# bblinn2017/inverse_path_tracer

Hardware: AMD Instinct MI355X
Metric: Msamples/sec fwd + grad-Msamples/sec, 512² Cornell 64spp, 1/2/4/8 GPU (higher is better)
Workload: dtype f32; 1 GPU; C2: CornellBox-Empty-CO.obj, 512x512, 64 spp, max_bounces=4; one frame per step tiled over the ranks as interleaved rows (fwd); adjoint dL/dKd of the rank's rows + RCCL all-reduce of the gradient (grad, --full); 3 frames in flight (consecutive steps round-robin over 3 HIP streams; one stream: secondary.serial); streams=3, width=512, height=512, spp=64, max_bounces=4, triangles=18, parallelism=interleaved row tiles x1

## Files before the change

inverse_path_tracer_amd/csrc/ipt_device.h:

```cpp
#pragma once
#include <hip/hip_runtime.h>
#include <stdint.h>

#include "scene_layout.h"

namespace ipt {
namespace dev {

typedef __attribute__((address_space(3))) float lds_f32;
typedef __attribute__((address_space(3))) double lds_f64;
typedef __attribute__((address_space(1))) float gbl_f32;
typedef __attribute__((address_space(1))) double gbl_f64;
typedef float v4f __attribute__((ext_vector_type(4)));
typedef __attribute__((address_space(3))) v4f lds_v4;
typedef __attribute__((address_space(1))) v4f gbl_v4;

constexpr float kMinDotUp = 0x1.a36e30p-14f;
constexpr float kEpsUp = 0x1.47ae16p-7f;
constexpr float kPRR = 0.9f;
constexpr float kPiF = 3.14159265358979323846f;
constexpr float kInvPiF = (float)(1.0 / 3.14159265358979323846);
constexpr double kPi = 3.14159265358979323846;

#ifndef IPT_DIV_CONST
// ... 1024 lines not shown
  if (M && lane == (int)__builtin_ctzll(__ballot(1))) atomicAdd(&g_bvh_stats[5], 1ull);
#endif
  while (M) {
#ifdef IPT_BVH_STATS
    if (lane == (int)__builtin_ctzll(__ballot(1))) atomicAdd(&g_bvh_stats[6], 1ull);
#endif
    uint64_t Mr = M;
    int src = -1;
#pragma unroll
    for (int k = 0; k < 8; ++k) {
      if (Mr) {
        const int idx = __builtin_ctzll(Mr);
        Mr &= Mr - 1;
        src = (g == k) ? idx : src;
      }
    }
    const uint64_t taken = M & ~Mr;
    M = Mr;
    const int sa = (src < 0 ? lane : src) << 2;
    const V3 gp = mk(bperm_f(sa, p.x), bperm_f(sa, p.y), bperm_f(sa, p.z));
    const V3 gd = mk(bperm_f(sa, d.x), bperm_f(sa, d.y), bperm_f(sa, d.z));
    float gt = bperm_f(sa, bt);
    int gi = __builtin_amdgcn_ds_bpermute(sa, bi);
    if (src >= 0) {
      coop_traverse<SHADOW>(C, gp, gd, gt, gi);
    }
    const int ra = (8 * lane_rank64(taken)) << 2;
    const float rt = bperm_f(ra, gt);
    const int ri = __builtin_amdgcn_ds_bpermute(ra, gi);
    if ((taken >> lane) & 1ull) {
      bt = rt;
      bi = ri;
    }
  }
}

__device__ __forceinline__ V3 shading_normal(const TriGeom &g, V3 q) {
  if (g.flags & GEOM_AXIS_FLAT) return mk(g.vn[0][0], g.vn[0][1], g.vn[0][2]);
  const V3 v0 = mk(g.v[0][0], g.v[0][1], g.v[0][2]);
  const V3 v1 = mk(g.v[1][0], g.v[1][1], g.v[1][2]);
  const V3 v2 = mk(g.v[2][0], g.v[2][1], g.v[2][2]);
  const V3 c0 = cross3(sub(v1, q), sub(v2, q));
  const V3 c1 = cross3(sub(v2, q), sub(v0, q));
  const V3 c2 = cross3(sub(v0, q), sub(v1, q));
  const float w0 = (0.5f * sqrtf(dot3(c0, c0))) / g.area;
  const float w1 = (0.5f * sqrtf(dot3(c1, c1))) / g.area;
  const float w2 = (0.5f * sqrtf(dot3(c2, c2))) / g.area;
  const V3 n = mk(fmaf(g.vn[2][0], w2, fmaf(g.vn[1][0], w1, g.vn[0][0] * w0)),
                  fmaf(g.vn[2][1], w2, fmaf(g.vn[1][1], w1, g.vn[0][1] * w0)),
                  fmaf(g.vn[2][2], w2, fmaf(g.vn[1][2], w1, g.vn[0][2] * w0)));
  return unit(n);
}

__device__ __forceinline__ void camera_ray(const float *cam, const float *org, Rng &st, int r, int c, int W, int H,
                                           float rcW, float rcH, V3 &p, V3 &d) {
  const float u0 = uniform(st), u1 = uniform(st);
  const float nx = 2.f * ((float)c + u0), ny = 2.f * ((float)r + u1);
  const float x = (rcW != 0.f ? nx * rcW : div_inrange(nx, (float)W)) - 1.f;
  const float y = 1.f - (rcH != 0.f ? ny * rcH : div_inrange(ny, (float)H));
  const V3 d0 = unit_in_range(mk(x, y, 1.f));
  float dr[3];
#pragma unroll
  for (int i = 0; i < 3; ++i) {
    const float *M = cam + 4 * i;
    dr[i] = fmaf(M[3], 0.f, fmaf(M[2], d0.z, fmaf(M[1], d0.y, M[0] * d0.x)));
  }
  p = mk(org[0], org[1], org[2]);
  d = unit(mk(dr[0], dr[1], dr[2]));
}

__device__ inline float phong(float shin, V3 nrm, V3 w, V3 wi) {
  const float dn = dot3(nrm, wi);
  const V3 refl = mk(fmaf(2.f * dn, nrm.x, -wi.x), fmaf(2.f * dn, nrm.y, -wi.y), fmaf(2.f * dn, nrm.z, -wi.z));
  const float pw = pow_f(dot3(refl, w), shin);
  const float mx = pw > 0.f ? pw : 0.f;
  return (float)((((double)(shin + 2.f)) / 2.0 / kPi) * (double)mx);
}

}
}
```

inverse_path_tracer_amd/csrc/ipt_hip.hip:

```cpp
#include <hip/hip_runtime.h>

#include <algorithm>
#include <atomic>
#include <cmath>
#include <cstdio>
#include <cstdlib>
#include <cstring>
#include <mutex>
#include <string>
#include <vector>

#include "bvh.h"
#include "gpu_api.h"
#include "ipt_device.h"

namespace ipt {

static thread_local std::string g_gpu_err;
void gpu_set_error(const std::string &e) { g_gpu_err = e; }
const char *gpu_last_error() { return g_gpu_err.c_str(); }
static std::atomic<int> g_fail_launches{0};
void gpu_debug_fail_launches(int n) { g_fail_launches.store(n > 0 ? n : 0); }
static std::atomic<int> g_adju_pool{0}, g_adju_lds{0};
void gpu_debug_adju_ring(int pool_chunks, int lds_slots) {
// ... 204 lines not shown
  return BVH || IPT_BF_BIG > 1;
}
template <bool GUIDED>
__device__ __forceinline__ void chunk_range(const TraceArgs &a, uint64_t g, uint64_t units, uint64_t &start,
                                            uint64_t &end) {
  const uint64_t nb = a.chunk_big_n;
  uint64_t len;
  if (!GUIDED || g < nb) {
    start = g * a.chunk;
    len = a.chunk;
  } else {
    start = nb * a.chunk + (g - nb) * a.chunk_small;
    len = a.chunk_small;
  }
  end = start + len < units ? start + len : units;
}

__device__ __forceinline__ void grab_failed(uint32_t *word, uint32_t c, uint32_t grabs) {
  if (c + 1u == grabs) __hip_atomic_store(word, 0u, __ATOMIC_RELAXED, __HIP_MEMORY_SCOPE_AGENT);
}

__device__ __forceinline__ uint64_t item_pixel(const TraceArgs &a, uint64_t w) {
  uint64_t lp, sj;
  item_split(a, w, lp, sj);
  int r, c;
  local_rc(a, lp, r, c);
  if (a.idx32) return (uint32_t)r * (uint32_t)a.W + (uint32_t)c;
  return (uint64_t)r * (uint64_t)a.W + (uint64_t)c;
}

using namespace dev;
typedef __attribute__((address_space(3))) uint32_t lds_u32;

__device__ __forceinline__ void item_ray_ls(const TraceArgs &a, uint64_t seed, uint64_t lp, uint64_t sj, Rng &st, V3 &p,
                                            V3 &d, int &r, int &c) {
  local_rc(a, lp, r, c);
  uint64_t g;
  if (a.idx32) {
    const uint32_t pixel = (uint32_t)r * (uint32_t)a.W + (uint32_t)c;
    g = (uint64_t)pixel * (uint32_t)a.spp + sj;
  } else {
    g = ((uint64_t)r * (uint64_t)a.W + (uint64_t)c) * (uint64_t)a.spp + sj;
  }
  rng_init(st, seed + g);
  camera_ray(a.cam, a.cam_org, st, r, c, a.W, a.H, a.rc_W, a.rc_H, p, d);
}
__device__ __forceinline__ void item_ray(const TraceArgs &a, uint64_t seed, uint64_t w, Rng &st, V3 &p, V3 &d, int &r,
                                         int &c) {
  uint64_t lp, sj;
  item_split(a, w, lp, sj);
  item_ray_ls(a, seed, lp, sj, st, p, d, r, c);
}

#ifndef IPT_MIN_BLOCKS_FWD
#define IPT_MIN_BLOCKS_FWD 5
#endif
#ifndef IPT_MIN_BLOCKS_ADJ
#define IPT_MIN_BLOCKS_ADJ 5
#endif
#ifndef IPT_MIN_BLOCKS_ADJU
#define IPT_MIN_BLOCKS_ADJU 5
#endif
#ifndef IPT_MIN_BLOCKS_ADJW
#define IPT_MIN_BLOCKS_ADJW 6
#endif
#ifndef IPT_ADJW_LANE_LDS
#define IPT_ADJW_LANE_LDS 1
#endif
#ifndef IPT_MIN_BLOCKS_GRAPH
#define IPT_MIN_BLOCKS_GRAPH 0
#endif
#ifndef IPT_MIN_BLOCKS_BVH
#define IPT_MIN_BLOCKS_BVH 4
#endif
#ifndef IPT_MIN_BLOCKS_BVH_ADJ
#define IPT_MIN_BLOCKS_BVH_ADJ 2
#endif
#ifndef IPT_MIN_BLOCKS_BVH_ADJU
#define IPT_MIN_BLOCKS_BVH_ADJU 4
#endif
#ifndef IPT_MIN_BLOCKS_BVH_FWD
#define IPT_MIN_BLOCKS_BVH_FWD 5
#endif
template <int MODE, bool BVH>
constexpr int min_blocks() {
  return BVH ? (MODE == MODE_ADJU ? IPT_MIN_BLOCKS_BVH_ADJU
                                  : (is_adj<MODE>() ? IPT_MIN_BLOCKS_BVH_ADJ
                                                    : (is_fwd<MODE>() ? IPT_MIN_BLOCKS_BVH_FWD : IPT_MIN_BLOCKS_BVH)))
             : (is_fwd<MODE>() ? IPT_MIN_BLOCKS_FWD
                                : (MODE == MODE_ADJU   ? IPT_MIN_BLOCKS_ADJU
                                   : MODE == MODE_ADJW ? IPT_MIN_BLOCKS_ADJW
                                                       : (is_adj<MODE>() ? IPT_MIN_BLOCKS_ADJ : IPT_MIN_BLOCKS_GRAPH)));
}
#ifndef IPT_GRAPH_LDS_KB
#define IPT_GRAPH_LDS_KB 64
#endif
#ifndef IPT_ADJ_PIXEL_MAJOR
#define IPT_ADJ_PIXEL_MAJOR 1
#endif
#ifndef IPT_GRAPH_PIXEL_MAJOR
#define IPT_GRAPH_PIXEL_MAJOR 1
#endif
#define IPT_TRACE_BOUNDS __attribute__((amdgpu_flat_work_group_size(1, kBlock), amdgpu_waves_per_eu(min_blocks<MODE, BVH>() ? min_blocks<MODE, BVH>() : 1)))
#ifdef IPT_PHASE_TIMING
constexpr int kPhaseWords = 26;
__device__ unsigned long long g_phase_cycles[kPhaseWords];
// ... 322 lines not shown
  if (hipMemcpyFromSymbol(out, HIP_SYMBOL(g_phase_cycles), kPhaseWords * sizeof(unsigned long long)) != hipSuccess)
    return -1;
  unsigned long long z[kPhaseWords] = {};
  return hipMemcpyToSymbol(HIP_SYMBOL(g_phase_cycles), z, sizeof z) == hipSuccess ? 0 : -1;
}
#endif

#ifdef IPT_BVH_STATS
extern "C" int ipt_debug_bvh_stats(unsigned long long *out) {
  if (hipMemcpyFromSymbol(out, HIP_SYMBOL(g_bvh_stats), kBvhStats * sizeof(unsigned long long)) != hipSuccess)
    return -1;
  unsigned long long z[kBvhStats] = {0};
  return hipMemcpyToSymbol(HIP_SYMBOL(g_bvh_stats), z, sizeof z) == hipSuccess ? 0 : -1;
}
#endif

const HostScene &gpu_host(const GpuScene *s) { return s->host; }
HostScene &gpu_host_mut(GpuScene *s) { return s->host; }

template <typename T>
static int upload(T **dst, const std::vector<T> &v) {
  const size_t n = std::max<size_t>(v.size(), 1) * sizeof(T);
  HIP_TRY(hipMalloc(reinterpret_cast<void **>(dst), n));
  if (!v.empty()) HIP_TRY(hipMemcpy(*dst, v.data(), v.size() * sizeof(T), hipMemcpyHostToDevice));
  return 0;
}

template <typename T>
static int upload_as_f4(float4 **dst, const std::vector<T> &v) {
  static_assert(sizeof(T) % sizeof(float4) == 0, "record is not a whole number of float4");
  HIP_TRY(hipMalloc(reinterpret_cast<void **>(dst), std::max<size_t>(v.size(), 1) * sizeof(T)));
  if (!v.empty()) HIP_TRY(hipMemcpy(*dst, v.data(), v.size() * sizeof(T), hipMemcpyHostToDevice));
  return 0;
}

static std::vector<float4> src_cull_f4(const HostScene &host) {
  std::vector<float4> v(host.bvh_src_cull.size() / 4);
  for (size_t i = 0; i < v.size(); ++i)
    v[i] = make_float4(host.bvh_src_cull[4 * i], host.bvh_src_cull[4 * i + 1], host.bvh_src_cull[4 * i + 2],
                       host.bvh_src_cull[4 * i + 3]);
  return v;
}

GpuScene *gpu_upload(const HostScene &host, std::string *err) {
  GpuScene *s = new GpuScene();
  s->host = host;
  if (hipGetDevice(&s->device) != hipSuccess) {
    *err = "no HIP device available";
    delete s;
    return nullptr;
  }
  std::vector<TriPair> pairs((host.isect.size() + 1) / 2);
  pack_pairs(host.isect.data(), (int)host.isect.size(), pairs.data());
  if (upload(&s->isect, host.isect) || upload(&s->pairs, pairs) || upload(&s->geom, host.geom) || upload(&s->mat, host.mat) ||
      upload(&s->kd, host.kd) || upload(&s->emit_tri, host.emit_tri) || upload(&s->emit_cdf, host.emit_cdf) ||
      upload(&s->emit_pmf, host.emit_pmf) || upload(&s->emit_pmfr, pmf_reciprocals(host.emit_pmf)) ||
      upload(&s->big_pairs, host.bvh_big_pairs) || upload(&s->big_idx, host.bvh_big_idx) ||
      upload(&s->big_boxes, host.bvh_big_boxes) ||
      upload_as_f4(&s->wide, host.bvh_wide) || upload(&s->src_cull, src_cull_f4(host)) ||
      upload(&s->wtris, host.bvh_wtris) || upload(&s->pboxes, pair_boxes(host)) ||
      upload(&s->pomask, shadow_occluder_masks(host)) ||
      upload(&s->big_pomask, host.bvh_big_idx.empty()
                                 ? std::vector<uint32_t>()
                                 : shadow_occluder_masks(host, std::vector<int>(host.bvh_big_idx.begin(),
                                                                                host.bvh_big_idx.end())))) {
    *err = gpu_last_error();
    gpu_free(s);
    return nullptr;
  }
  for (const TriMat &m : host.mat) s->has_ks |= (m.flags & MAT_HAS_KS) != 0;
  {
    std::vector<int> te((size_t)host.nT, -1);
    for (int e = 0; e < host.nE; ++e) te[(size_t)host.emit_tri[(size_t)e]] = e;
    if (upload(&s->tri_emit, te)) {
      *err = gpu_last_error();
      gpu_free(s);
      return nullptr;
    }
  }
  {
    hipMemPool_t pool;
    if (hipDeviceGetDefaultMemPool(&pool, s->device) == hipSuccess) {
      uint64_t keep = ~0ull;
      (void)hipMemPoolSetAttribute(pool, hipMemPoolAttrReleaseThreshold, &keep);
    }
  }
  if ((size_t)host.nT * 3 * sizeof(double) > (size_t)kLdsGradBytes) {
    const int slots = kLdsGradBytes / (3 * (int)sizeof(double));
    std::vector<int> order(host.nT), map(host.nT, -1), inv(slots);
    for (int i = 0; i < host.nT; ++i) order[i] = i;
    std::stable_sort(order.begin(), order.end(),
                     [&](int x, int y) { return host.geom[(size_t)x].area > host.geom[(size_t)y].area; });
    for (int k = 0; k < slots; ++k) {
      map[(size_t)order[(size_t)k]] = k;
      inv[(size_t)k] = order[(size_t)k];
    }
    if (upload(&s->grad_map, map) || upload(&s->slot_tri, inv)) {
      *err = gpu_last_error();
      gpu_free(s);
      return nullptr;
    }
  }
  s->on_device = true;
  return s;
}

GpuScene *gpu_host_only(const HostScene &host) {
// ... 518 lines not shown
  return pixel_mean_sm_sets(samples_dev, npix, spp, 1, hdr_dev, ldr_dev, stream);
}

#ifndef IPT_FUSED_MEAN
#define IPT_FUSED_MEAN 1
#endif
#ifndef IPT_FUSED_GRAB_SAMPLES
#define IPT_FUSED_GRAB_SAMPLES 256
#endif
#ifndef IPT_FUSED_WAVE_BYTES
#define IPT_FUSED_WAVE_BYTES 6144
#endif
struct FusedShape {
  int slots, group, per_grab;
};
#ifndef IPT_FUSED_BVH
#define IPT_FUSED_BVH 0
#endif
#ifndef IPT_FUSED_BVH_WAVE_BYTES
#define IPT_FUSED_BVH_WAVE_BYTES 3072
#endif
static FusedShape fused_shape(const RenderParams &p, bool bvh) {
  const FusedShape none = {0, 0, 0};
  if (!IPT_FUSED_MEAN || !IPT_DYN_CHUNKS) return none;
  if ((uint64_t)p.width * (uint64_t)p.height * (uint64_t)p.spp > 0xffffffffull || p.spp > 256) return none;
  int bytes = IPT_FUSED_WAVE_BYTES;
  if (bvh) {
    if (!IPT_FUSED_BVH) return none;
    bytes = IPT_FUSED_BVH_WAVE_BYTES;
  }
  const int slots = std::min(16, bytes / (12 * p.spp));
  const bool long_paths = p.max_bounces < 0 || p.max_bounces > 8;
  const int cap = slots / (long_paths ? 4 : 2);
  if (cap < 1) return none;
  int g = 1;
  while (2 * g <= cap && 2 * g * p.spp <= 256) g *= 2;
  if (g * p.spp < 32) return none;
  const int per_grab = std::min(8, (IPT_FUSED_GRAB_SAMPLES + g * p.spp - 1) / (g * p.spp));
  return {slots, g, per_grab};
}

static int render_impl(GpuScene *s, const RenderParams &p, const float *kd_dev, float *hdr_dev, uint8_t *ldr_dev,
                       void *stream, const TriMat *mat_dev) {
  if (check_params(s, p)) return -1;
  const int64_t npix = (int64_t)band_rows(p) * p.width;
  const int sets = p.nscenes > 1 ? p.nscenes : 1;
  const FusedShape fs = fused_shape(p, use_bvh(s));
  if (fs.group > 0) {
    TraceArgs a = make_args(s, p);
    a.fused = 1;
    a.group = (uint32_t)fs.group;
    a.chunk = (uint32_t)(fs.group * fs.per_grab);
    a.nslots = fs.slots;
    a.mean_wstride = (uint32_t)(((2 * fs.slots + 3) & ~3) + 3 * fs.slots * p.spp + 3) & ~3u;
    a.ldr = ldr_dev;
    a.out_stride = (uint64_t)npix * 3;
    const size_t tail = (size_t)(kBlock / 64) * a.mean_wstride * sizeof(float);
    return launch<MODE_FWDM>(s, a, table_bytes(a), kd_dev, hdr_dev, nullptr, nullptr, nullptr, nullptr,
                             (hipStream_t)stream, tail, mat_dev);
  }
  StreamScratch ws;
  if (ws.alloc((size_t)sets * npix * p.spp * 3 * sizeof(float), (hipStream_t)stream)) return -1;
  if (render_samples_sm(s, p, kd_dev, (float *)ws.p, stream, mat_dev)) return -1;
  return pixel_mean_sm_sets((const float *)ws.p, npix, p.spp, sets, hdr_dev, ldr_dev, stream);
}
int gpu_render(GpuScene *s, const RenderParams &p, const float *kd_dev, float *hdr_dev, uint8_t *ldr_dev,
               void *stream) {
  return render_impl(s, p, kd_dev, hdr_dev, ldr_dev, stream, nullptr);
}

int gpu_set_material_params(GpuScene *s, const float *kd, const float *ks, const float *ke) {
  HostScene &h = s->host;
  if (kd) std::memcpy(h.kd.data(), kd, h.kd.size() * sizeof(float));
  std::vector<char> em((size_t)h.nT, 0);
  for (int e : h.emit_tri) em[(size_t)e] = 1;
  for (int i = 0; i < h.nT; ++i) {
    TriMat &m = h.mat[(size_t)i];
    for (int c = 0; c < 3; ++c) {
      if (ks) m.ks[c] = (m.flags & MAT_HAS_KS) ? ks[3 * i + c] : 0.f;
      if (ke) m.ke[c] = em[(size_t)i] ? ke[3 * i + c] : 0.f;
    }
  }
  if (!s->on_device) return 0;
  if (kd) HIP_TRY(hipMemcpy(s->kd, h.kd.data(), h.kd.size() * sizeof(float), hipMemcpyHostToDevice));
  if (ks || ke) HIP_TRY(hipMemcpy(s->mat, h.mat.data(), h.mat.size() * sizeof(TriMat), hipMemcpyHostToDevice));
  return 0;
}

static int pack_materials(GpuScene *s, const float *ks_dev, const float *ke_dev, int sets, hipStream_t st,
                          StreamScratch &buf, const TriMat **mat) {
  *mat = nullptr;
  if (!ks_dev && !ke_dev) return 0;
  const int nT = s->host.nT;
  if (buf.alloc((size_t)sets * nT * sizeof(TriMat), st)) return -1;
  hipLaunchKernelGGL(pack_mat_kernel, dim3((nT + kBlock - 1) / kBlock, sets), dim3(kBlock), 0, st, s->mat, ks_dev,
                     ke_dev, s->tri_emit, nT, (TriMat *)buf.p);
  HIP_TRY(hipGetLastError());
  *mat = (const TriMat *)buf.p;
  return 0;
}

static int batch_kd(GpuScene *s, const float **kd_dev, int sets, hipStream_t st, StreamScratch &buf) {
  if (*kd_dev || sets <= 1) return 0;
  const int n = 3 * s->host.nT;
  const size_t total = (size_t)sets * n;
  if (buf.alloc(total * sizeof(float), st)) return -1;
  hipLaunchKernelGGL(replicate_kernel, dim3((unsigned)((total + kBlock - 1) / kBlock)), dim3(kBlock), 0, st, s->kd, n,
// ... 633 lines not shown
```

inverse_path_tracer_amd/csrc/trace_body.h:

```cpp
  extern __shared__ double lds[];
  const int tid = threadIdx.x;
  const int set = a.nscenes > 1 ? (int)(blockIdx.x % (uint32_t)a.nscenes) : 0;
  const uint32_t sblock = a.nscenes > 1 ? blockIdx.x / (uint32_t)a.nscenes : blockIdx.x;
  const uint32_t sgrid = a.nscenes > 1 ? (uint32_t)a.bps : gridDim.x;
  const uint64_t seed = a.seed + (uint64_t)set * a.seed_stride;
  if (a.nscenes > 1) {
    kd += (size_t)set * 3 * a.nT;
    if (MATG || MATB) mat += (size_t)set * a.mat_stride;
    if (is_fwd<MODE>()) out_samples += (size_t)set * a.out_stride;
  }
  const float *kdpi_g = a.kdpi_g ? a.kdpi_g + (size_t)set * 3 * a.nT : nullptr;
  constexpr int nthr = kBlock;
  const int nT = a.nT, nE = a.nE;
  const int vmax = a.rec_cap;
  double *lds_acc = lds;
  int n_acc = 0;
  if (is_adj<MODE>()) {
    n_acc = a.grad_slots * 3;
    if (MATG) n_acc = (int)mat_lds_doubles(a.grad_slots, nE, SPEC);
  } else if (MODE == MODE_GRAPH && a.lds_edges) {
    n_acc = (int)graph_lds_doubles(nT, nE);
  }
  float *tab = reinterpret_cast<float *>(lds + n_acc);
  if (a.kd_tables) {
// ... 167 lines not shown
  };
  auto carry_put3 = [&](int f, V3 v) {
    lds_f32 *w = (lds_f32 *)carry_at(f, tid);
    w[0] = v.x;
    w[kBlock] = v.y;
    w[2 * kBlock] = v.z;
  };
  auto carry_get3 = [&](int f, int l) -> V3 {
    const lds_f32 *w = (const lds_f32 *)carry_at(f, (tid & ~63) + l);
    return mk(w[0], w[kBlock], w[2 * kBlock]);
  };
  int usub = 0;
  auto pending = [&]() { return MODE == MODE_ADJU && kSub > 0 && usub > 0; };
  constexpr uint32_t kNoChunks = 0x00ffffffu;
  uint32_t ctab = kNoChunks | ((uint32_t)vmax << 24);
  uint64_t pfree = MODE == MODE_ADJU ? (a.pool_chunks >= 64 ? ~0ull : (1ull << a.pool_chunks) - 1ull) : 0ull;
  auto vcap_of = [&]() { return (int)(ctab >> 24); };
  float weight = 1.f;
  V3 pix = p;
  int k = 0, dst = 0;
  int ptri_r = -1;
  uint64_t witem_r = 0;
  auto set_item = [&](uint64_t w) {
    if (kLaneLds) {
      lane_ws[tid] = (uint32_t)w;
      lane_ws[kBlock + tid] = (uint32_t)(w >> 32);
    } else if (kCarryLds) {
      lds_u32 *q = carry_at(7, tid);
      q[0] = (uint32_t)w;
      q[kBlock] = (uint32_t)(w >> 32);
    } else {
      witem_r = w;
    }
  };
  auto witem = [&]() -> uint64_t {
    if (kLaneLds) return (uint64_t)lane_ws[tid] | ((uint64_t)lane_ws[kBlock + tid] << 32);
    if (kCarryLds) {
      const lds_u32 *q = carry_at(7, tid);
      return (uint64_t)q[0] | ((uint64_t)q[kBlock] << 32);
    }
    return witem_r;
  };
  auto set_ptri = [&](int t) {
    if (!BVH) return;
    if (kLaneLds) lane_ws[2 * kBlock + tid] = (uint32_t)t;
    else ptri_r = t;
  };
  auto ptri = [&]() -> int { return kLaneLds ? (int)lane_ws[2 * kBlock + tid] : ptri_r; };
#ifdef IPT_PHASE_TIMING
  uint64_t tacc[kPhaseWords] = {};
  uint64_t tp_ = __builtin_amdgcn_s_memtime();
#endif
  const int lane = tid & 63;
  auto fused_tab = [&](const TraceArgs &A) -> lds_u32 * {
    return (lds_u32 *)(reinterpret_cast<char *>(lds) + A.mean_off) + (size_t)(tid >> 6) * A.mean_wstride;
  };
  auto fused_slots = [&](const TraceArgs &A) -> lds_f32 * {
    return (lds_f32 *)(fused_tab(A) + ((2 * A.nslots + 3) & ~3));
  };
  auto fused_sum = [&](const TraceArgs &A, uint32_t mask) {
    __builtin_amdgcn_fence(__ATOMIC_RELEASE, "wavefront");
    __builtin_amdgcn_wave_barrier();
    const int m = __popc(mask);
    const int kq = (lane * 43) >> 7;
    int ch = lane - 3 * kq;
    asm volatile("" : "+v"(ch));
    int slot = 0;
    uint32_t mm = mask;
    for (int i = 0; i < m; ++i) {
      const int b = __builtin_ctz(mm);
      mm &= mm - 1u;
      slot = kq == i ? b : slot;
    }
    if (lane < 3 * m) {
      const int spp = A.spp;
      const lds_f32 *v = fused_slots(A) + (size_t)(3 * slot + ch) * spp;
      float acc = 0.f;
      if (A.rc_spp != 0.f && (spp & 3) == 0) {
        const float rc = A.rc_spp;
        for (int s = 0; s < spp; s += 4) {
          const v4f w4 = *(const lds_v4 *)(v + s);
          acc += w4.x * rc;
          acc += w4.y * rc;
          acc += w4.z * rc;
          acc += w4.w * rc;
        }
      } else {
        const float fs = (float)spp;
        for (int s = 0; s < spp; ++s) acc += v[s] / fs;
      }
      const uint64_t px = fused_tab(A)[A.nslots + slot];
      out_samples[px * 3 + ch] = acc;
      if (A.ldr) A.ldr[(size_t)set * A.out_stride + px * 3 + ch] = (uint8_t)(255.f * acc / (1 + acc));
    }
    __builtin_amdgcn_fence(__ATOMIC_RELEASE, "wavefront");
    __builtin_amdgcn_wave_barrier();
  };
  for (;;) {
#if defined(__HIP_DEVICE_COMPILE__)
    typedef __attribute__((address_space(4))) const TraceArgs cst_args;
    const cst_args *apc = (const cst_args *)__builtin_amdgcn_kernarg_segment_ptr();
    asm volatile("" : "+s"(apc));
    TraceArgs a = *apc;
#else
    TraceArgs a = ar;
#endif
    if (MODE == MODE_FWDM) {
      const uint32_t G = a.group;
      const bool issued = fj >= gnp * (uint32_t)a.spp;
      if (sdone && ((uint32_t)__popc(sdone) >= G || exhausted || (issued && (uint32_t)__popc(sfree) < G))) {
        fused_sum(a, sdone);
        sfree |= sdone;
        sdone = 0;
      }
      if (issued && !exhausted && (uint32_t)__popc(sfree) >= G) {
        if (pl0 >= pl1) {
          bool own = false;
          if (!started) {
            started = true;
            chunk_range<kGuided<BVH>()>(a, wave, a.npix, pl0, pl1);
            own = pl0 < a.npix;
          }
          if (!own) {
            uint32_t c = 0;
            if (lane == 0) c = atomicAdd(a.chunk_ctr + (size_t)set * kCtrStride, 1u);
            c = (uint32_t)__builtin_amdgcn_readfirstlane((int)c);
            chunk_range<kGuided<BVH>()>(a, nwaves + c, a.npix, pl0, pl1);
            if (pl0 >= a.npix && lane == 0) grab_failed(a.chunk_ctr + (size_t)set * kCtrStride, c, a.grabs);
          }
        }
        if (pl0 < a.npix) {
          glp = (uint32_t)pl0;
          gnp = (uint32_t)(pl1 - pl0 < G ? pl1 - pl0 : G);
          pl0 += gnp;
          fj = 0;
          gslots = 0;
          uint32_t mm = sfree;
          for (uint32_t q = 0; q < gnp; ++q) {
            gslots |= (uint32_t)__builtin_ctz(mm) << (4 * q);
            mm &= mm - 1u;
          }
          sfree = mm;
          if ((uint32_t)lane < gnp) {
            lds_u32 *tab = fused_tab(a);
            const uint32_t sl = (gslots >> (4 * lane)) & 15u;
            tab[sl] = (uint32_t)a.spp;
            tab[a.nslots + sl] = glp + (uint32_t)lane;
          }
        } else {
          exhausted = true;
        }
      }
    } else if (next >= end && !exhausted) {
      uint32_t c = 0;
      if (lane == 0) c = atomicAdd(a.chunk_ctr + (size_t)set * kCtrStride, 1u);
      c = (uint32_t)__shfl((int)c, 0);
      uint64_t start, stop;
      chunk_range<kGuided<BVH>()>(a, nwaves + c, a.n_samples, start, stop);
      if (start < a.n_samples) {
        next = start;
        end = stop;
      } else {
        exhausted = true;
        if (lane == 0) grab_failed(a.chunk_ctr + (size_t)set * kCtrStride, c, a.grabs);
      }
    }
    const bool wants = !active && !pending();
    const uint64_t need = __ballot(wants);
#ifdef IPT_PHASE_TIMING
    const uint64_t act0_ = ~need;
#endif
    if (MODE == MODE_FWDM) {
      const uint32_t fn = gnp * (uint32_t)a.spp;
      if (need && fj < fn) {
        const uint32_t rank =
            __builtin_amdgcn_mbcnt_hi((uint32_t)(need >> 32), __builtin_amdgcn_mbcnt_lo((uint32_t)need, 0u));
        if (!active && fj + rank < fn) {
          const uint32_t j = fj + rank;
          const uint32_t s = (gnp & (gnp - 1u)) == 0u ? j >> __builtin_ctz(gnp) : j / gnp;
          const uint32_t q = j - s * gnp;
          int r, c;
          item_ray_ls(a, seed, glp + q, s, st, p, d, r, c);
          set_item((uint64_t)((gslots >> (4 * q)) & 15u) | ((uint64_t)s << 4));
          L = mk(0.f, 0.f, 0.f);
          set_le(L);
          Ld = L;
          M = mk(1.f, 1.f, 1.f);
          k = 0;
          set_ptri(-1);
          active = true;
        }
        fj += (uint32_t)__popcll(need);
        fj = fj < fn ? fj : fn;
      }
    } else if (need) {
      const uint32_t rank =
          __builtin_amdgcn_mbcnt_hi((uint32_t)(need >> 32), __builtin_amdgcn_mbcnt_lo((uint32_t)need, 0u));
      if (wants) {
        const uint64_t w = next + rank;
        if (w < end) {
          set_item(w);
          int r, c;
          item_ray(a, seed, w, st, p, d, r, c);
          L = mk(0.f, 0.f, 0.f);
          set_le(L);
          Ld = L;
          M = mk(1.f, 1.f, 1.f);
          k = 0;
          set_ptri(-1);
          if (MODE == MODE_ADJU) {
            rhi = 0;
            rslot = 0;
            if (!kSub) Mlo = mk(1.f, 1.f, 1.f);
            ctab = kNoChunks | ((uint32_t)vmax << 24);
          }
          if (MODE == MODE_GRAPH) {
            weight = 1.f;
            dst = nT;
            const uint8_t *px = target + ((size_t)r * a.W + c) * 3;
            pix = mk((float)px[0] / 255.0f, (float)px[1] / 255.0f, (float)px[2] / 255.0f);
          }
          active = true;
        }
      }
      next += (uint64_t)__popcll(need);
    }
    PHASE(0)
    PHASE_LANES(10, active && !((act0_ >> (tid & 63)) & 1ull))
    if (__ballot(active || pending()) == 0 &&
        (MODE != MODE_FWDM || (exhausted && sdone == 0 && fj >= gnp * (uint32_t)a.spp)))
      break;
#ifdef IPT_PHASE_TIMING
    tacc[6] += 1;
    tacc[7] += __popcll(__ballot(active));
#endif

    float t = 0.f;
    int hit = -1;
    if (BVH) {
      bool qn = false;
      if (active) {
        bvh_prepass<false>(bv, p, d, t, hit, -1);
        qn = coop_root_test(cv, p, d, t) && !(IPT_TREE_SKIP && tree_skip(a.src_cull, ptri(), d));
      }
      SUBPHASE_BEGIN
      coop_cast<false>(cv, qn, p, d, t, hit);
      SUBPHASE_END(8)
    } else if (active) {
      if (IPT_PATH_CULL && e3)
        hit = closest_hit_pairs_culled((const lds_f32 *)lds_pr, a.pboxes, nT, p, d, t);
      else
        hit = cast_bf(pairs, e3, nT, p, d, t);
    }
    PHASE(1)
    const bool vertex = active && hit >= 0;
    bool finished = false, escaped = false;
    if (active && hit < 0) {
      finished = true;
      escaped = (k > 0);
      if (MODE != MODE_GRAPH) {
        const V3 Le = le();
        L = mk(fmaf(M.x, Le.x + Ld.x, L.x), fmaf(M.y, Le.y + Ld.y, L.y), fmaf(M.z, Le.z + Ld.z, L.z));
      }
    }
    const int tri = hit;
    V3 nh = p, din = d, sd = d, nd = d;
    bool shadow = false, cont = false;
    int emitter = 0;
    float ct = 0.f, coeff = 0.f, speci = 0.f, specd = 0.f;
    if (vertex) {
      const V3 q = along(p, d, t);
      if (MODE == MODE_GRAPH) {
        (void)uniform(st);
        const float wf = weight * 1.f;
        const double v[5] = {(double)weight, (double)wf, (double)(wf * pix.x), (double)(wf * pix.y),
                             (double)(wf * pix.z)};
        const size_t bin = (size_t)dst * nT + tri;
        bins_add(a.lds_edges != 0, edges, a.lds_edges ? bin * kEdgeL : bin * kEdgeW, 5, v);
      } else if (k == 0) {
        set_le(ke3(tri));
        if (kTri0Carry) {
          if (kCarryLds) *carry_at(6, tid) = (uint32_t)tri;
          else tri0_r = tri;
        }
      }
      nh = shading_normal(geom[tri], q);
      p = q;
      Ld = mk(0.f, 0.f, 0.f);
      if (nE > 0) {
        const float u = uniform(st);
        int ie = 0;
        while (ie < nE && !(emit_cdf[ie] >= u)) ++ie;
        ie = ie < nE ? ie : nE - 1;
        const float r1 = uniform(st), r2 = uniform(st);
        const double sq = dsqrt_core((double)r1);
        const float ca = (float)(1.0 - sq);
        const float cb = (float)(sq * (double)(1.f - r2));
        const float cc = (float)((double)r2 * sq);
        const TriGeom &ge = geom[emit_tri[ie]];
        const V3 pt = mk(fmaf(cc, ge.v[2][0], fmaf(cb, ge.v[1][0], ca * ge.v[0][0])),
                         fmaf(cc, ge.v[2][1], fmaf(cb, ge.v[1][1], ca * ge.v[0][1])),
                         fmaf(cc, ge.v[2][2], fmaf(cb, ge.v[1][2], ca * ge.v[0][2])));
        sd = unit(sub(pt, q));
        ct = dot3(nh, sd);
        emitter = ie;
        shadow = !(ct < 0.f);
      }
      if (!(a.max_bounces >= 0 && k == a.max_bounces)) {
        const float pr = uniform(st);
        if (pr < kPRR) {
          const TriMat &m = mat[tri];
          const bool spec = SPEC && (MODE != MODE_GRAPH) && (m.flags & MAT_SPECULAR);
          const float uphi = uniform(st);
          const float phi = (float)(2.0 * kPi * (double)uphi);
          const float ut = uniform(st);
          float cth, sth, psamp;
          if (!spec) {
            cth = sqrt_core(ut);
            const float omu = 1.0f - ut;
            sth = omu > 0.f ? sqrt_core(omu) : 0.f;
            psamp = kInvPiF;
          } else {
            const double cd = pow_d((double)ut, 1.0 / ((double)m.shininess + 1.0));
            cth = (float)cd;
            sth = (float)sqrt(1.0 - cd * cd);
            psamp = pow_f((m.shininess + 1.f) * cth, m.shininess);
          }
          float sp, cp;
          sincos_f(phi, sp, cp);
          const V3 h = mk(sth * cp, sth * sp, cth);
          const TriGeom &g = geom[tri];
          nd = unit(mk(fmaf(g.R[0][2], h.z, fmaf(g.R[0][1], h.y, g.R[0][0] * h.x)),
                       fmaf(g.R[1][2], h.z, fmaf(g.R[1][1], h.y, g.R[1][0] * h.x)),
                       fmaf(g.R[2][2], h.z, fmaf(g.R[2][1], h.y, g.R[2][0] * h.x))));
          if (MODE != MODE_GRAPH) {
            if (SPEC && (m.flags & MAT_HAS_KS)) speci = phong(m.shininess, nh, din, nd);
            coeff = spec ? (dot3(nd, nh) / psamp) / kPRR : div_const<1>(div_const<0>(dot3(nd, nh)));
          }
          cont = true;
        }
      }
    }

    PHASE(2)
    PHASE_LANES(12, vertex)
    V3 lo = mk(0.f, 0.f, 0.f);
    float emit_s = 0.f;
    int emit_et = 0;
    float ts = 0.f;
    int hs = -1;
    const int et = shadow ? emit_tri[emitter] : -1;
    if (__ballot(shadow)) {
      PHASE_LANES(14, shadow)
      if (BVH) {
        bool qn = false;
        if (shadow && bvh_prepass<true>(bv, p, sd, ts, hs, et,
                                        a.big_pomask ? a.big_pomask[tri * nE + emitter] : 0xffffffffu, emitter))
          qn = coop_root_test(cv, p, sd, ts) && !(IPT_TREE_SKIP && tree_skip(a.src_cull, tri, sd));
        SUBPHASE_BEGIN
        coop_cast<true>(cv, qn, p, sd, ts, hs);
        SUBPHASE_END(9)
      } else if (shadow) {
        if (IPT_SHADOW_CULL && e3)
          hs = shadow_hit_pairs_small((const lds_f32 *)(IPT_SHADOW_PAIR1 ? lds_pr : lds_is), pairs, a.pboxes, e3, nT, p, sd, et, ts,
                                      [&]() { return po ? ((const lds_u32c *)lds_po)[tri * nE + emitter] : 0xffffffffu; });
        else
          hs = cast_bf(pairs, e3, nT, p, sd, ts);
      }
      PHASE(3)
      if (shadow && hs == et) {
        const V3 ne = shading_normal(geom[et], along(p, sd, ts));
        const float ctp = -dot3(ne, sd);
        if (!(ctp < 0.f)) {
          const double td = (double)ts;
          const TriMat &me = mat[et];
          if (MODE == MODE_GRAPH) {
            const double q = (double)((weight * ct) * ctp) / (td * td), pr = a.emit_pmfr[emitter];
            double w2d;
            if (pr != 0.0)
              w2d = q * pr;
            else
              w2d = q / (double)emit_pmf[emitter];
            const float w2 = (float)w2d;
            const float wf = w2 * kInvPiF;
            const double v[8] = {(double)w2, (double)wf, (double)(wf * pix.x), (double)(wf * pix.y),
                                 (double)(wf * pix.z), (double)(wf * me.ke[0]), (double)(wf * me.ke[1]),
                                 (double)(wf * me.ke[2])};
            const size_t bin = (size_t)tri * nT + et;
            if (a.lds_edges) {
              bins_add(true, edges, bin * kEdgeL, 5, v);
              bins_add(true, edges, (size_t)(nT + 1) * nT * kEdgeL + ((size_t)tri * nE + emitter) * 3, 3, v + 5);
// ... 90 lines not shown
        if (kSub > 0) {
          if (rslot % kSub == 0 && k > 0) {
            gbl_f32 *m = umr + (size_t)(rslot / kSub) * 192;
            m[0] = M.x;
            m[1] = M.y;
            m[2] = M.z;
          }
        } else if (rslot == 0) {
          if (kCarryLds) carry_put3(3, M);
          else Mlo = M;
        }
        rslot = (rslot + 1 == vcap_of()) ? 0 : rslot + 1;
      }
      if (MODE == MODE_GRAPH) {
        if (cont) {
          weight *= dot3(nd, nh);
          weight = (float)((double)weight * (((1.0 / (double)kInvPiF) / (double)kPRR) / 1.0));
          dst = tri;
        }
      } else {
        const V3 Le = le();
        L = mk(fmaf(M.x, Le.x + Ld.x, L.x), fmaf(M.y, Le.y + Ld.y, L.y), fmaf(M.z, Le.z + Ld.z, L.z));
        if (cont) {
          const V3 tp = kdpi3(tri);
          const float t0 = tp.x, t1 = tp.y, t2 = tp.z;
          if (SPEC) {
            const TriMat &m = mat[tri];
            M = mk((M.x * (t0 + m.ks[0] * speci)) * coeff, (M.y * (t1 + m.ks[1] * speci)) * coeff,
                   (M.z * (t2 + m.ks[2] * speci)) * coeff);
          } else {
            M = mk((M.x * t0) * coeff, (M.y * t1) * coeff, (M.z * t2) * coeff);
          }
        }
      }
      ++k;
      if (BVH) set_ptri(tri);
      if (cont) d = nd;
      else finished = true;
      if (MODE == MODE_ADJU && rhi > 0 && k == rhi) finished = true;
    }

    int uhi = 0, ulo = 0, urep = 0;
    bool uend = false, uesc = false;
    const bool upend = pending();
    if (upend) {
      uhi = usub;
      ulo = rhi == 0 ? k - (rslot == 0 ? vcap_of() : rslot) : rhi - vcap_of();
      if (ulo > 0) urep = ulo;
    }
    if (finished) {
      active = false;
      if (MODE == MODE_FWDM) {
        const uint64_t wi = witem();
        lds_f32 *o = fused_slots(a) + (uint32_t)(wi & 15u) * 3u * (uint32_t)a.spp + (uint32_t)(wi >> 4);
        o[0] = L.x;
        o[a.spp] = L.y;
        o[2 * a.spp] = L.z;
      } else if (MODE == MODE_FWD) {
        float *o = out_samples + witem() * 3;
        o[0] = L.x;
        o[1] = L.y;
        o[2] = L.z;
      } else if (MODE == MODE_ADJU) {
        if (rhi == 0) {
          uhi = k;
          ulo = k > 0 ? k - (rslot == 0 ? vcap_of() : rslot) : 0;
          uend = true;
          uesc = escaped;
        } else {
          uhi = rhi;
          ulo = rhi - vcap_of();
        }
        if (ulo > 0) urep = ulo;
      }
    }
    const int uslo = (MODE == MODE_ADJU && kSub > 0 && uhi > ulo) ? ulo + kSub * ((uhi - 1 - ulo) / kSub) : ulo;
    if (MODE == MODE_FWDM && __ballot(finished)) {
      __builtin_amdgcn_fence(__ATOMIC_RELEASE, "wavefront");
      __builtin_amdgcn_wave_barrier();
      uint32_t left = 0;
      if (finished)
        left = __hip_atomic_fetch_sub(fused_tab(a) + (uint32_t)(witem() & 15u), 1u, __ATOMIC_RELAXED,
                                      __HIP_MEMORY_SCOPE_WORKGROUP);
      uint64_t comp = __ballot(finished && left == 1u);
      while (comp) {
        const int l = (int)__builtin_ctzll(comp);
        comp &= comp - 1ull;
        sdone |= 1u << (__builtin_amdgcn_readlane((int)(witem() & 15u), l) & 31);
      }
    }
    if (is_adj<MODE>()) {
      const int Kf = is_badj<MODE>() ? ((finished && k > 0) ? k : 0) : (uhi > 0 ? uhi - uslo : 0);
      if (__ballot(Kf > 0)) {
        const int lane = tid & 63;
        const int inc = wave_scan_add(Kf);
        const int T = __builtin_amdgcn_readlane(inc, 63);
        uint32_t *swl = reinterpret_cast<uint32_t *>(lds_rec) - kBlock + (tid & ~63);
        float wx = 0.f, wy = 0.f, wz = 0.f;
        if (Kf > 0) {
          const float *adj = karg<const float *>(offsetof(TraceKernArgs, adj)) +
                             (a.nscenes > 1 ? (size_t)set * a.adj_stride : 0);
          const uint64_t pixel = item_pixel(a, witem());
          if (a.rc_spp != 0.f) {
            wx = adj[pixel * 3 + 0] * a.rc_spp;
            wy = adj[pixel * 3 + 1] * a.rc_spp;
            wz = adj[pixel * 3 + 2] * a.rc_spp;
          } else {
            wx = adj[pixel * 3 + 0] / (float)a.spp;
            wy = adj[pixel * 3 + 1] / (float)a.spp;
            wz = adj[pixel * 3 + 2] / (float)a.spp;
          }
        }
        const size_t fs = (size_t)vmax * kBlock;
        int base = 0;
        while (base < T) {
          const uint64_t fit = __ballot(Kf > 0 && inc <= base + 64);
          const int next = __builtin_amdgcn_readlane(inc, 63 - (int)__builtin_clzll(fit));
          const int t = base + lane;
          const bool valid = t < next;
          PHASE_LANES(20, valid)
          swl[lane] = 0u;
          const int st0 = inc - Kf - base;
          const bool owns = Kf > 0 && inc <= next && st0 >= 0;
          const bool oend = is_badj<MODE>() || uend, oesc = is_badj<MODE>() ? escaped : uesc;
          if (owns)
            swl[st0] = (((uint32_t)st0 << 21) | ((uint32_t)(MODE == MODE_ADJU ? uslo - ulo : 0) << 15) |
                        (oend ? 1u << 14 : 0u) | (oesc ? 1u << 13 : 0u) | ((uint32_t)Kf << 6) | (uint32_t)lane) + 1u;
          __builtin_amdgcn_fence(__ATOMIC_RELEASE, "wavefront");
          __builtin_amdgcn_wave_barrier();
          const uint32_t mk_ = wave_scan_max(swl[lane]) - 1u;
          __builtin_amdgcn_fence(__ATOMIC_RELEASE, "wavefront");
          __builtin_amdgcn_wave_barrier();
          const int ow = valid ? (int)(mk_ & 63u) : lane;
          const int KL = valid ? (int)((mk_ >> 6) & 127u) : 0;
          const int kk = valid ? lane - (int)(mk_ >> 21) : 0;
          const bool esc = valid && ((mk_ >> 13) & 1u);
          const bool fst_o = is_badj<MODE>() || (valid && ((mk_ >> 14) & 1u));
          const int rr = valid ? KL - 1 - kk : 0;
          const V3 Lev = le();
          V3 LeL = mk(__shfl(Lev.x, ow), __shfl(Lev.y, ow), __shfl(Lev.z, ow));
          if (kCarryLds) {
            __builtin_amdgcn_fence(__ATOMIC_RELEASE, "wavefront");
// ... 265 lines not shown
```

Measured before the change: 11880 Msamples/s.

## Refill finished paths in-phase with camera rays sharing the bounce sampling code

In the fused forward kernel without BVH, lanes whose path ends at this bounce are immediately given a new camera sample within the same iteration. The camera direction is generated through the same sample-and-rotate code as the BSDF continuation, using a camera rotation stored as an extra TriGeom entry. Per-pixel RNG base and row/column are precomputed into LDS entries when a group is grabbed, so the refill only adds a sample index. The goal is to cut divergence and idle lanes between the separate refill phase and the bounce phase, at the cost of extra LDS per wave and more control-flow complexity.

```diff
diff --git a/inverse_path_tracer_amd/csrc/ipt_device.h b/inverse_path_tracer_amd/csrc/ipt_device.h
--- a/inverse_path_tracer_amd/csrc/ipt_device.h
+++ b/inverse_path_tracer_amd/csrc/ipt_device.h
@@ -1100,21 +1100,29 @@
   return unit(n);
 }
 
+__device__ __forceinline__ V3 camera_local(float u0, float u1, float cf, float rf, int W, int H, float rcW, float rcH) {
+  const float nx = 2.f * (cf + u0), ny = 2.f * (rf + u1);
+  const float x = (rcW != 0.f ? nx * rcW : div_inrange(nx, (float)W)) - 1.f;
+  const float y = 1.f - (rcH != 0.f ? ny * rcH : div_inrange(ny, (float)H));
+  return unit_in_range(mk(x, y, 1.f));
+}
+__device__ __forceinline__ V3 rotate3(const float *R0, const float *R1, const float *R2, V3 h) {
+  return mk(fmaf(R0[2], h.z, fmaf(R0[1], h.y, R0[0] * h.x)), fmaf(R1[2], h.z, fmaf(R1[1], h.y, R1[0] * h.x)),
+            fmaf(R2[2], h.z, fmaf(R2[1], h.y, R2[0] * h.x)));
+}
+__device__ __forceinline__ V3 camera_w0(const float *cam, V3 v) {
+  return mk(fmaf(cam[3], 0.f, v.x), fmaf(cam[7], 0.f, v.y), fmaf(cam[11], 0.f, v.z));
+}
+__device__ __forceinline__ void camera_ray_f(const float *cam, const float *org, Rng &st, float rf, float cf, int W, int H,
+                                             float rcW, float rcH, V3 &p, V3 &d) {
+  const float u0 = uniform(st), u1 = uniform(st);
+  const V3 d0 = camera_local(u0, u1, cf, rf, W, H, rcW, rcH);
+  p = mk(org[0], org[1], org[2]);
+  d = unit(camera_w0(cam, rotate3(cam, cam + 4, cam + 8, d0)));
+}
 __device__ __forceinline__ void camera_ray(const float *cam, const float *org, Rng &st, int r, int c, int W, int H,
                                            float rcW, float rcH, V3 &p, V3 &d) {
-  const float u0 = uniform(st), u1 = uniform(st);
-  const float nx = 2.f * ((float)c + u0), ny = 2.f * ((float)r + u1);
-  const float x = (rcW != 0.f ? nx * rcW : div_inrange(nx, (float)W)) - 1.f;
-  const float y = 1.f - (rcH != 0.f ? ny * rcH : div_inrange(ny, (float)H));
-  const V3 d0 = unit_in_range(mk(x, y, 1.f));
-  float dr[3];
-#pragma unroll
-  for (int i = 0; i < 3; ++i) {
-    const float *M = cam + 4 * i;
-    dr[i] = fmaf(M[3], 0.f, fmaf(M[2], d0.z, fmaf(M[1], d0.y, M[0] * d0.x)));
-  }
-  p = mk(org[0], org[1], org[2]);
-  d = unit(mk(dr[0], dr[1], dr[2]));
+  camera_ray_f(cam, org, st, (float)r, (float)c, W, H, rcW, rcH, p, d);
 }
 
 __device__ inline float phong(float shin, V3 nrm, V3 w, V3 wi) {
diff --git a/inverse_path_tracer_amd/csrc/ipt_hip.hip b/inverse_path_tracer_amd/csrc/ipt_hip.hip
--- a/inverse_path_tracer_amd/csrc/ipt_hip.hip
+++ b/inverse_path_tracer_amd/csrc/ipt_hip.hip
@@ -280,6 +280,43 @@
   item_ray_ls(a, seed, lp, sj, st, p, d, r, c);
 }
 
+#ifndef IPT_INPHASE_REFILL
+#define IPT_INPHASE_REFILL 1
+#endif
+#ifndef IPT_INPHASE_MERGE
+#define IPT_INPHASE_MERGE 1
+#endif
+#ifndef IPT_INPHASE_PACK
+#define IPT_INPHASE_PACK 0
+#endif
+template <int MODE, bool BVH>
+constexpr bool kInphase() {
+  return IPT_INPHASE_REFILL && MODE == MODE_FWDM && !BVH;
+}
+constexpr int kEntryWords = 4;
+static inline uint32_t fused_entry_words(uint32_t group, bool bvh) {
+  return (IPT_INPHASE_REFILL && !bvh) ? kEntryWords * group : 0u;
+}
+__device__ __forceinline__ void pixel_entry(const TraceArgs &a, uint64_t seed, uint64_t lp, uint32_t e[kEntryWords]) {
+  int r, c;
+  local_rc(a, lp, r, c);
+  uint64_t g0;
+  if (a.idx32) {
+    const uint32_t pixel = (uint32_t)r * (uint32_t)a.W + (uint32_t)c;
+    g0 = (uint64_t)pixel * (uint32_t)a.spp;
+  } else {
+    g0 = ((uint64_t)r * (uint64_t)a.W + (uint64_t)c) * (uint64_t)a.spp;
+  }
+  g0 += seed;
+  e[0] = (uint32_t)g0;
+  e[1] = (uint32_t)(g0 >> 32);
+  e[2] = __float_as_uint((float)c);
+  e[3] = __float_as_uint((float)r);
+}
+#ifndef IPT_REFILL_ABLATE
+#define IPT_REFILL_ABLATE 0
+#endif
+
 #ifndef IPT_MIN_BLOCKS_FWD
 #define IPT_MIN_BLOCKS_FWD 5
 #endif
@@ -708,7 +745,11 @@
   }
   std::vector<TriPair> pairs((host.isect.size() + 1) / 2);
   pack_pairs(host.isect.data(), (int)host.isect.size(), pairs.data());
-  if (upload(&s->isect, host.isect) || upload(&s->pairs, pairs) || upload(&s->geom, host.geom) || upload(&s->mat, host.mat) ||
+  std::vector<TriGeom> geom(host.geom);
+  geom.resize((size_t)host.nT + 1, TriGeom());
+  for (int i = 0; i < 3; ++i)
+    for (int j = 0; j < 3; ++j) geom[(size_t)host.nT].R[i][j] = host.cam[4 * i + j];
+  if (upload(&s->isect, host.isect) || upload(&s->pairs, pairs) || upload(&s->geom, geom) || upload(&s->mat, host.mat) ||
       upload(&s->kd, host.kd) || upload(&s->emit_tri, host.emit_tri) || upload(&s->emit_cdf, host.emit_cdf) ||
       upload(&s->emit_pmf, host.emit_pmf) || upload(&s->emit_pmfr, pmf_reciprocals(host.emit_pmf)) ||
       upload(&s->big_pairs, host.bvh_big_pairs) || upload(&s->big_idx, host.bvh_big_idx) ||
@@ -1333,7 +1374,8 @@
     a.group = (uint32_t)fs.group;
     a.chunk = (uint32_t)(fs.group * fs.per_grab);
     a.nslots = fs.slots;
-    a.mean_wstride = (uint32_t)(((2 * fs.slots + 3) & ~3) + 3 * fs.slots * p.spp + 3) & ~3u;
+    a.mean_wstride = (uint32_t)(((2 * fs.slots + 3) & ~3) + fused_entry_words((uint32_t)fs.group, use_bvh(s)) +
+                                3 * fs.slots * p.spp + 3) & ~3u;
     a.ldr = ldr_dev;
     a.out_stride = (uint64_t)npix * 3;
     const size_t tail = (size_t)(kBlock / 64) * a.mean_wstride * sizeof(float);
diff --git a/inverse_path_tracer_amd/csrc/trace_body.h b/inverse_path_tracer_amd/csrc/trace_body.h
--- a/inverse_path_tracer_amd/csrc/trace_body.h
+++ b/inverse_path_tracer_amd/csrc/trace_body.h
@@ -243,11 +243,23 @@
   uint64_t tp_ = __builtin_amdgcn_s_memtime();
 #endif
   const int lane = tid & 63;
+  constexpr bool kInph = kInphase<MODE, BVH>();
+  constexpr bool kInphM = kInph && IPT_INPHASE_MERGE;
+  constexpr bool kInphP = kInphM && (SPEC || IPT_INPHASE_PACK);
   auto fused_tab = [&](const TraceArgs &A) -> lds_u32 * {
     return (lds_u32 *)(reinterpret_cast<char *>(lds) + A.mean_off) + (size_t)(tid >> 6) * A.mean_wstride;
   };
+  auto fused_entries = [&](const TraceArgs &A) -> lds_u32 * { return fused_tab(A) + ((2 * A.nslots + 3) & ~3); };
   auto fused_slots = [&](const TraceArgs &A) -> lds_f32 * {
-    return (lds_f32 *)(fused_tab(A) + ((2 * A.nslots + 3) & ~3));
+    return (lds_f32 *)(fused_tab(A) + ((2 * A.nslots + 3) & ~3) + (kInph ? kEntryWords * A.group : 0u));
+  };
+  auto entry_sample = [&](const TraceArgs &A, uint32_t q, uint32_t s, float &cf, float &rf) -> uint64_t {
+    typedef uint32_t v4u __attribute__((ext_vector_type(4)));
+    typedef __attribute__((address_space(3))) v4u lds_v4u;
+    const v4u e = *(const lds_v4u *)(fused_entries(A) + kEntryWords * q);
+    cf = __uint_as_float(e.z);
+    rf = __uint_as_float(e.w);
+    return (((uint64_t)e.y << 32) | (uint64_t)e.x) + (uint64_t)s;
   };
   auto fused_sum = [&](const TraceArgs &A, uint32_t mask) {
     __builtin_amdgcn_fence(__ATOMIC_RELEASE, "wavefront");
@@ -337,6 +349,17 @@
             const uint32_t sl = (gslots >> (4 * lane)) & 15u;
             tab[sl] = (uint32_t)a.spp;
             tab[a.nslots + sl] = glp + (uint32_t)lane;
+            if (kInph) {
+              uint32_t e[kEntryWords];
+              pixel_entry(a, seed, glp + (uint32_t)lane, e);
+              lds_u32 *w = fused_entries(a) + kEntryWords * lane;
+#pragma unroll
+              for (int i = 0; i < kEntryWords; ++i) w[i] = e[i];
+            }
+          }
+          if (kInph) {
+            __builtin_amdgcn_fence(__ATOMIC_RELEASE, "wavefront");
+            __builtin_amdgcn_wave_barrier();
           }
         } else {
           exhausted = true;
@@ -370,9 +393,31 @@
           const uint32_t j = fj + rank;
           const uint32_t s = (gnp & (gnp - 1u)) == 0u ? j >> __builtin_ctz(gnp) : j / gnp;
           const uint32_t q = j - s * gnp;
-          int r, c;
-          item_ray_ls(a, seed, glp + q, s, st, p, d, r, c);
-          set_item((uint64_t)((gslots >> (4 * q)) & 15u) | ((uint64_t)s << 4));
+          if (IPT_REFILL_ABLATE && !BVH) {
+            uint64_t g = (uint64_t)(glp * (uint32_t)a.spp + j);
+            if (IPT_REFILL_ABLATE < 2) {
+              int r, c;
+              local_rc(a, glp + q, r, c);
+              g = (uint64_t)((uint32_t)r * (uint32_t)a.W + (uint32_t)c) * (uint32_t)a.spp + s;
+            }
+            rng_init(st, seed + g);
+            p = mk(a.cam_org[0], a.cam_org[1], a.cam_org[2]);
+            d = mk(a.cam[2], a.cam[6], a.cam[10]);
+            if (IPT_REFILL_ABLATE == 3) {
+              const float u0 = uniform(st), u1 = uniform(st);
+              d = mk(2.f * ((float)((glp + q) & 511u) + u0) * a.rc_W - 1.f,
+                     1.f - 2.f * ((float)((glp + q) >> 9) + u1) * a.rc_H, 1.f);
+            }
+          } else if (kInph) {
+            float cf, rf;
+            rng_init(st, entry_sample(a, q, s, cf, rf));
+            camera_ray_f(a.cam, a.cam_org, st, rf, cf, a.W, a.H, a.rc_W, a.rc_H, p, d);
+          } else {
+            int r, c;
+            item_ray_ls(a, seed, glp + q, s, st, p, d, r, c);
+          }
+          if (kInph) set_item((uint64_t)(((gslots >> (4 * q)) & 15u) | (s << 4)));
+          else set_item((uint64_t)((gslots >> (4 * q)) & 15u) | ((uint64_t)s << 4));
           L = mk(0.f, 0.f, 0.f);
           set_le(L);
           Ld = L;
@@ -457,6 +502,8 @@
     const int tri = hit;
     V3 nh = p, din = d, sd = d, nd = d;
     bool shadow = false, cont = false;
+    bool wantc = false, refill = false;
+    uint32_t nitem = 0;
     int emitter = 0;
     float ct = 0.f, coeff = 0.f, speci = 0.f, specd = 0.f;
     if (vertex) {
@@ -499,7 +546,9 @@
       }
       if (!(a.max_bounces >= 0 && k == a.max_bounces)) {
         const float pr = uniform(st);
-        if (pr < kPRR) {
+        if (kInphM) {
+          wantc = pr < kPRR;
+        } else if (pr < kPRR) {
           const TriMat &m = mat[tri];
           const bool spec = SPEC && (MODE != MODE_GRAPH) && (m.flags & MAT_SPECULAR);
           const float uphi = uniform(st);
@@ -528,6 +577,63 @@
             if (SPEC && (m.flags & MAT_HAS_KS)) speci = phong(m.shininess, nh, din, nd);
             coeff = spec ? (dot3(nd, nh) / psamp) / kPRR : div_const<1>(div_const<0>(dot3(nd, nh)));
           }
+          cont = true;
+        }
+      }
+    }
+    if (kInphM) {
+      const bool ends = active && !wantc;
+      const uint64_t ask = __ballot(ends);
+      const uint32_t fn = gnp * (uint32_t)a.spp;
+      float ecf = 0.f, erf = 0.f;
+      if (ask && fj < fn) {
+        const uint32_t rank =
+            __builtin_amdgcn_mbcnt_hi((uint32_t)(ask >> 32), __builtin_amdgcn_mbcnt_lo((uint32_t)ask, 0u));
+        if (ends && fj + rank < fn) {
+          const uint32_t j = fj + rank;
+          const uint32_t s = (gnp & (gnp - 1u)) == 0u ? j >> __builtin_ctz(gnp) : j / gnp;
+          const uint32_t q = j - s * gnp;
+          rng_init(st, entry_sample(a, q, s, ecf, erf));
+          nitem = ((gslots >> (4 * q)) & 15u) | (s << 4);
+          if (kInphP) set_item(witem() | (uint64_t)((nitem | 0x1000u) << 16));
+          refill = true;
+        }
+        fj += (uint32_t)__popcll(ask);
+        fj = fj < fn ? fj : fn;
+      }
+      if (wantc || refill) {
+        const float ua = uniform(st);
+        const float ub = uniform(st);
+        const TriMat &m = mat[refill ? 0 : tri];
+        const bool spec = SPEC && !refill && (m.flags & MAT_SPECULAR);
+        float psamp = kInvPiF;
+        V3 h;
+        if (refill) {
+          h = camera_local(ua, ub, ecf, erf, a.W, a.H, a.rc_W, a.rc_H);
+        } else {
+          const float phi = (float)(2.0 * kPi * (double)ua);
+          float cth, sth;
+          if (!spec) {
+            cth = sqrt_core(ub);
+            const float omu = 1.0f - ub;
+            sth = omu > 0.f ? sqrt_core(omu) : 0.f;
+          } else {
+            const double cd = pow_d((double)ub, 1.0 / ((double)m.shininess + 1.0));
+            cth = (float)cd;
+            sth = (float)sqrt(1.0 - cd * cd);
+            psamp = pow_f((m.shininess + 1.f) * cth, m.shininess);
+          }
+          float sp, cp;
+          sincos_f(phi, sp, cp);
+          h = mk(sth * cp, sth * sp, cth);
+        }
+        const TriGeom &g = geom[refill ? nT : tri];
+        V3 v = rotate3(g.R[0], g.R[1], g.R[2], h);
+        if (refill) v = camera_w0(a.cam, v);
+        nd = unit(v);
+        if (wantc) {
+          if (SPEC && (m.flags & MAT_HAS_KS)) speci = phong(m.shininess, nh, din, nd);
+          coeff = spec ? (dot3(nd, nh) / psamp) / kPRR : div_const<1>(div_const<0>(dot3(nd, nh)));
           cont = true;
         }
       }
@@ -724,7 +830,8 @@
       active = false;
       if (MODE == MODE_FWDM) {
         const uint64_t wi = witem();
-        lds_f32 *o = fused_slots(a) + (uint32_t)(wi & 15u) * 3u * (uint32_t)a.spp + (uint32_t)(wi >> 4);
+        lds_f32 *o = fused_slots(a) + (uint32_t)(wi & 15u) * 3u * (uint32_t)a.spp +
+                     (kInphP ? ((uint32_t)wi >> 4) & 0xffu : (uint32_t)(wi >> 4));
         o[0] = L.x;
         o[a.spp] = L.y;
         o[2 * a.spp] = L.z;
@@ -760,6 +867,17 @@
         comp &= comp - 1ull;
         sdone |= 1u << (__builtin_amdgcn_readlane((int)(witem() & 15u), l) & 31);
       }
+    }
+    if (kInphM && (kInphP ? ((uint32_t)witem() >> 16) != 0u : refill)) {
+      L = mk(0.f, 0.f, 0.f);
+      set_le(L);
+      Ld = L;
+      M = mk(1.f, 1.f, 1.f);
+      k = 0;
+      p = mk(a.cam_org[0], a.cam_org[1], a.cam_org[2]);
+      d = nd;
+      set_item(kInphP ? (uint64_t)(((uint32_t)witem() >> 16) & 0xfffu) : (uint64_t)nitem);
+      active = true;
     }
     if (is_adj<MODE>()) {
       const int Kf = is_badj<MODE>() ? ((finished && k > 0) ? k : 0) : (uhi > 0 ? uhi - uslo : 0);
```

After: 12120 Msamples/s (median of 6 runs). 1.02x the previous value.
